# theodorblackbird/lina-speech

Hardware: AMD Instinct MI355X
Metric: codec tokens/sec (whole node), 169M d1024xl12 batched greedy decode (higher is better)
Workload: dtype bf16

## Files before the change

### include/lina_gla.h

```cpp
#ifndef LINA_GLA_H
#define LINA_GLA_H

#include <stdint.h>

#ifdef __cplusplus
extern "C" {
#endif

typedef void* lina_stream_t;

enum { LINA_F32 = 0, LINA_BF16 = 1 };
enum {
    LINA_OK = 0,
    LINA_ERR_ARG = -1,
    LINA_ERR_UNSUPPORTED = -2,
    LINA_ERR_LAUNCH = -3
};

int lina_version(void);
const char* lina_last_error(void);

typedef struct lina_bht_strides {
    int64_t b, h, t;
} lina_bht_strides;
// ... 178 lines not shown
                           float* state, const void* gate, const void* norm_weight,
                           void* og, float* o_exchange, int* counters,
                           float* hist_k, float* hist_c, float* hist_v,
                           const int64_t* step, const int64_t* origin, int window,
                           int B, int H, int Dk, int Dv,
                           int64_t q_sb, int64_t q_sh, int64_t k_sb, int64_t k_sh,
                           int64_t v_sb, int64_t v_sh, int64_t g_sb, int64_t g_sh,
                           int64_t gate_sb, int64_t gate_sh, float eps, int og_packed,
                           int dtype, int g_dtype, float scale, lina_stream_t stream);
int lina_gla_decode_window_flush(float* state, const float* hist_k, const float* hist_c, const float* hist_v,
                                 int n_pending, int B, int H, int Dk, int Dv, lina_stream_t stream);
int lina_gla_decode_window_s(const void* q, const void* k, const void* v, const void* gk,
                             void* state, int state_dtype, const void* gate, const void* norm_weight,
                             void* og, float* o_exchange, int* counters,
                             float* hist_k, float* hist_c, float* hist_v,
                             const int64_t* step, const int64_t* origin, int window,
                             int B, int H, int Dk, int Dv,
                             int64_t q_sb, int64_t q_sh, int64_t k_sb, int64_t k_sh,
                             int64_t v_sb, int64_t v_sh, int64_t g_sb, int64_t g_sh,
                             int64_t gate_sb, int64_t gate_sh, float eps, int og_packed,
                             int dtype, int g_dtype, float scale, lina_stream_t stream);
int lina_gla_decode_window_flush_s(void* state, int state_dtype, const float* hist_k, const float* hist_c,
                                   const float* hist_v, int n_pending, int B, int H, int Dk, int Dv, lina_stream_t stream);

int lina_linear_skinny(const void* A, int64_t lda, const void* W, int64_t ldw,
                       const float* c1, const float* c2, const void* resid, int64_t ldr,
                       void* out, int64_t ldo, int M, int N, int K,
                       int swiglu_hidden, int ln_dim, float ln_eps, int dtype, lina_stream_t stream);

int lina_gla_decode_inproj(const void* x, int64_t ldx, const void* w_in, int64_t ldw,
                           const float* c1, const float* c2,
                           const void* wq, const void* wk, const void* wv,
                           void* cq, void* ck, void* cv, const void* w2, const void* b2,
                           void* qkv, void* g_out, float* gk,
                           int B, int K, int Kd, int Vd, int W, int R,
                           float ln_eps, float normalizer, float clamp_min, int dtype, lina_stream_t stream);

int lina_cross_att_step1(const void* q_lin, const void* ln_w, const void* ln_b, float ln_eps,
                         const void* kk, const void* pe, void* att1, int64_t att_sb, void* xp,
                         int B, int T_txt, int d, float scale, int dtype, lina_stream_t stream);
int lina_cross_att_step2(const void* xp, const void* pe, const void* vv, void* att2, int64_t att_sb, void* x,
                         int B, int T_txt, int d, float scale, int dtype, lina_stream_t stream);

int lina_softmax_pe_rows(const float* scores, int64_t scores_sb, void* att, int64_t att_sb,
                         const int64_t* att_step, int64_t att_step_stride, int64_t att_steps, const void* pe, void* xp,
                         void* xp_packed, int B, int Tn, int d, int dtype, lina_stream_t stream);
// ... 42 lines not shown
```

### lina-speech_amd/_lib.py

```python
from __future__ import annotations

import ctypes as C
import os

_HERE = os.path.dirname(os.path.abspath(__file__))
LIB_PATH = os.environ.get("LINA_GLA_LIB") or os.path.join(_HERE, "csrc", "liblina_gla.so")

LINA_F32, LINA_BF16 = 0, 1
CONV_BWD_TT = 64
LOOP_CTL_ROWS = 4


class BHT(C.Structure):
    _fields_ = [("b", C.c_int64), ("h", C.c_int64), ("t", C.c_int64)]


_p, _i, _i64, _f = C.c_void_p, C.c_int, C.c_int64, C.c_float

_GLA_SIG = [_p, _p, _p, _p, _p, _p, _p, _i, _i, _i, _i, _i, BHT, BHT, BHT, BHT, BHT, _i, _i, _f, _p]

PROTOTYPES = {
    "lina_version": (C.c_int, []),
    "lina_last_error": (C.c_char_p, []),
    "lina_gla_recurrent_fwd": (C.c_int, _GLA_SIG),
# ... 29 lines not shown
    "lina_sum_partials": (C.c_int, [_p, _p, _i, _i, _i64, _i, _p]),
    "lina_mlp_pack": (C.c_int, [_p, _p, _p, _p, _p, _p, _p, _i, _i, _i, _i, _i, _i, _p]),
    "lina_stack_rows": (C.c_int, [_p, _p, _i, _i, _i, _p, _i, _p]),
    "lina_adamw_multi": (C.c_int, [_p, _p, _p, _p, _p, _i] + [C.c_double] * 7 + [_p]),
    "lina_adamw_multi_max": (C.c_int, []),
    "lina_swiglu_bwd_partials": (C.c_int, [_i64]),
    "lina_swiglu_bwd_colsum": (C.c_int, [_p, _p, _p, _p, _i64, _i, _i64, _i64, _i64, _i, _p]),
    "lina_gate_lowrank_partials": (C.c_int, [_i64]),
    "lina_gate_lowrank": (C.c_int, [_p, _i64, _p, _p, _p, _p, _p, _i64, _i, _i, _f, _f, _i, _p]),
    "lina_gate_logsigmoid": (C.c_int, [_p, _p, _p, _i64, _f, _f, _i, _p]),
    "lina_layernorm_fwd": (C.c_int, [_p, _p, _p, _p, _p, _p, _p, _p, _i64, _i, _f, _i, _i, _i, _p]),
    "lina_layernorm_bwd_partials": (C.c_int, [_i64]),
    "lina_layernorm_bwd": (C.c_int, [_p, _p, _p, _p, _p, _p, _p, _p, _p, _p, _i64, _i, _i, _i, _i, _p]),
    "lina_gla_decode_update": (C.c_int, [_p, _p, _p, _p, _p, _p, _i, _i, _i, _i, _i64, _i64, _i64, _i64, _i64, _i64,
                                         _i64, _i64, _i, _i, _f, _p]),
    "lina_gla_decode_update_norm": (C.c_int, [_p, _p, _p, _p, _p, _p, _p, _p, _p, _p, _i, _i, _i, _i,
                                              _i64, _i64, _i64, _i64, _i64, _i64, _i64, _i64, _i64, _i64, _f,
                                              _i, _i, _f, _p]),
    "lina_gla_decode_window_max": (C.c_int, []),
    "lina_gla_decode_window": (C.c_int, [_p] * 15 + [_i] * 5 + [_i64] * 10 + [_f, _i, _i, _i, _f, _p]),
    "lina_gla_decode_window_flush": (C.c_int, [_p, _p, _p, _p, _i, _i, _i, _i, _i, _p]),
    "lina_gla_decode_window_s": (C.c_int, [_p] * 5 + [_i] + [_p] * 10 + [_i] * 5 + [_i64] * 10 + [_f, _i, _i, _i, _f, _p]),
    "lina_gla_decode_window_flush_s": (C.c_int, [_p, _i, _p, _p, _p, _i, _i, _i, _i, _i, _p]),
    "lina_linear_skinny_ex": (C.c_int, [_p, _i64, _p, _i64, _i, _i, _p, _p, _p, _i64, _p, _i64, _p, _i, _i, _i, _i, _i, _i, _f, _i, _p]),
    "lina_gla_decode_inproj_packed": (C.c_int, [_p] * 15 + [_i] * 6 + [_f, _f, _f, _i, _i, _p]),
    "lina_weighted_rows_add_packed": (C.c_int, [_p, _i, _p, _p, _p, _i, _i, _i, _i, _p]),
    "lina_cross_att_step1": (C.c_int, [_p, _p, _p, _f, _p, _p, _p, _i64, _p, _i, _i, _i, _f, _i, _p]),
    "lina_cross_att_step2": (C.c_int, [_p, _p, _p, _p, _i64, _p, _i, _i, _i, _f, _i, _p]),
    "lina_cross_scores_softmax": (C.c_int, [_p, _p, _p, _f, _p, _p, _i64, _p, _i, _i, _i, _i, _f, _i, _p]),
    "lina_softmax_weighted_rows_add": (C.c_int, [_p, _i64, _f, _p, _i64, _p, _p, _p, _i, _i, _i, _i, _p]),
    "lina_pe_softmax_weighted_rows_add": (C.c_int, [_p, _i, _p, _f, _p, _i64, _p, _i64, _i64, _p, _p, _p, _i, _i, _i, _i, _p]),
    "lina_softmax_pe_rows": (C.c_int, [_p, _i64, _p, _i64, _p, _i64, _i64, _p, _p, _p, _i, _i, _i, _i, _p]),
    "lina_cross_scores": (C.c_int, [_p, _p, _p, _f, _p, _p, _i, _i, _i, _f, _i, _p]),
    "lina_cross_scores_ragged": (C.c_int, [_p, _p, _p, _f, _p, _p, _p, _i, _i, _i, _f, _i, _p]),
    "lina_softmax_pe_rows_ragged": (C.c_int, [_p, _i64, _p, _i64, _p, _i64, _i64, _p, _i64, _p, _p, _p, _i, _i, _i, _i, _p]),
    "lina_pe_softmax_weighted_rows_add_ragged": (C.c_int, [_p, _i, _p, _i64, _p, _f, _p, _i64, _p, _i64, _i64, _p, _p, _p,
                                                           _i, _i, _i, _i, _p]),
    "lina_softmax_rows": (C.c_int, [_p, _i64, _i, _f, _p, _i64, _p, _i, _i, _i, _i, _p]),
    "lina_weighted_rows_add": (C.c_int, [_p, _i, _p, _p, _i, _i, _i, _i, _p]),
    "lina_gla_decode_inproj": (C.c_int, [_p, _i64, _p, _i64, _p, _p, _p, _p, _p, _p, _p, _p, _p, _p, _p, _p, _p,
                                         _i, _i, _i, _i, _i, _i, _f, _f, _f, _i, _p]),
    "lina_linear_skinny": (C.c_int, [_p, _i64, _p, _i64, _p, _p, _p, _i64, _p, _i64, _i, _i, _i, _i, _i, _f, _i, _p]),
}


def _preload_hip_runtime() -> None:
# ... 44 lines not shown
```

### lina-speech_amd/csrc/gla_decode_window.hip

```cpp
#include <lina_dev.h>
#include "lina_common.h"
#include "skinny_frag.h"

#ifndef LINA_K1W_HIST_NT
#define LINA_K1W_HIST_NT 0
#endif

#ifndef LINA_K1W_STATE_PLAIN
#define LINA_K1W_STATE_PLAIN 0
#endif
#ifndef LINA_K1W_NO_TAIL_LOADS
#define LINA_K1W_NO_TAIL_LOADS 0
#endif
#if LINA_K1W_STATE_PLAIN
#define LINA_K1W_STATE_LOAD(p) (*reinterpret_cast<const float4*>(p))
#else
#define LINA_K1W_STATE_LOAD(p) ld_nt4(p)
#endif

namespace lina {

constexpr int kWinMax = 16;

__device__ __forceinline__ float ld_hist(const float* p) {
// ... 238 lines not shown
                float4 oth[CS];
                float tot = ss;
#pragma unroll
                for (int c = 0; c < CS; ++c) {
                    oth[c] = r;
                    if (c != (int)blockIdx.y) {
                        float4 x = make_float4(0.f, 0.f, 0.f, 0.f);
                        if (tid < CG4) {
                            const float2 lo = ld_agent8(ox + c * DV + 4 * tid), hi = ld_agent8(ox + c * DV + 4 * tid + 2);
                            x = make_float4(lo.x, lo.y, hi.x, hi.y);
                        }
                        float s2 = x.x * x.x + x.y * x.y + x.z * x.z + x.w * x.w;
                        s2 += shfl_xor(s2, 1); s2 += shfl_xor(s2, 2); s2 += shfl_xor(s2, 4);
                        s2 += shfl_xor(s2, 8); s2 += shfl_xor(s2, 16); s2 += shfl_xor(s2, 32);
                        tot += s2;
                        oth[c] = x;
                    }
                }
                const float rs = rsqrtf(tot / (float)DVT + eps);
#pragma unroll
                for (int c = 0; c < CS; ++c) finish(oth[c], c * DV, rs);
            }
        }
    }
}

template <typename TIO, typename TG, typename TS = float>
static int launch_window(const void* q, const void* k, const void* v, const void* gk, TS* S, float* hk, float* hc,
                         float* hv, const int64_t* step, const int64_t* origin, int window, int flush_n, int B, int H,
                         int Dk, int Dv, const int64_t* st, float scale, lina_stream_t stream, const void* gate,
                         int64_t gate_sb, int64_t gate_sh, const void* nw, float eps, void* og, int og_packed = 0,
                         float* o_x = nullptr, int* counters = nullptr) {
    const int cs = Dv == 512 ? 2 : 1;
    dim3 grid((unsigned)(B * H), (unsigned)cs);
#define LINA_WIN_ONE(DVV, NRBB, CSS)                                                                                   \
    LINA_LAUNCH((gla_decode_window_kernel<DVV, NRBB, CSS, TIO, TG, TS>), grid, dim3(256 * NRBB), 0, stream, (const TIO*)q, \
                (const TIO*)k, (const TIO*)v, (const TG*)gk, S, hk, hc, hv, step, origin, window, flush_n, H, st[0],   \
                st[1], st[2], st[3], st[4], st[5], st[6], st[7], scale, (const TIO*)gate, gate_sb, gate_sh,            \
                (const TIO*)nw, eps, (TIO*)og, og_packed, o_x, counters)
#define LINA_WIN_CASE(DVV)                                                                                             \
    case DVV:                                                                                                          \
        if (Dk == 64) LINA_WIN_ONE(DVV, 1, 1); else if (Dk == 128) LINA_WIN_ONE(DVV, 2, 1); else LINA_WIN_ONE(DVV, 4, 1); \
        break;
    if (Dk != 64 && Dk != 128 && Dk != 256)
        return fail(LINA_ERR_UNSUPPORTED, "lina_gla_decode_window: Dk=%d not in {64,128,256}", Dk);
    if (cs == 2 && flush_n < 0 && !(o_x && counters))
        return fail(LINA_ERR_ARG, "lina_gla_decode_window: Dv=512 needs the o_exchange buffer and the counters");
    switch (Dv) {
        LINA_WIN_CASE(64) LINA_WIN_CASE(128) LINA_WIN_CASE(256)
        case 512:
            if (Dk == 64) LINA_WIN_ONE(256, 1, 2); else if (Dk == 128) LINA_WIN_ONE(256, 2, 2); else LINA_WIN_ONE(256, 4, 2);
            break;
        default: return fail(LINA_ERR_UNSUPPORTED, "lina_gla_decode_window: Dv=%d not in {64,128,256,512}", Dv);
    }
#undef LINA_WIN_CASE
#undef LINA_WIN_ONE
    return check_launch("lina_gla_decode_window");
}

}

extern "C" int lina_gla_decode_window_max(void) { return lina::kWinMax; }

extern "C" int lina_gla_decode_window(const void* q, const void* k, const void* v, const void* gk,
                                      float* state, const void* gate, const void* norm_weight, void* og,
                                      float* o_exchange, int* counters, float* hist_k, float* hist_c, float* hist_v, const int64_t* step,
                                      const int64_t* origin, int window, int B, int H, int Dk, int Dv, int64_t q_sb,
                                      int64_t q_sh, int64_t k_sb, int64_t k_sh, int64_t v_sb, int64_t v_sh, int64_t g_sb,
                                      int64_t g_sh, int64_t gate_sb, int64_t gate_sh, float eps, int og_packed, int dtype,
                                      int g_dtype, float scale, lina_stream_t stream) {
    using namespace lina;
    LINA_REQUIRE(q && k && v && gk && state && gate && norm_weight && og && hist_k && hist_c && hist_v && step && origin,
                 "lina_gla_decode_window: null pointer");
    LINA_REQUIRE(B > 0 && H > 0, "lina_gla_decode_window: B,H must be positive");
    LINA_REQUIRE(window >= 1 && window <= kWinMax && (window & (window - 1)) == 0,
                 "lina_gla_decode_window: window must be a power of two in [1, %d]", kWinMax);
    LINA_REQUIRE(valid_dtype(dtype) && valid_dtype(g_dtype), "lina_gla_decode_window: bad dtype enum");
    LINA_REQUIRE(gate_sb % 4 == 0 && gate_sh % 4 == 0, "lina_gla_decode_window: gate strides must be multiples of 4");
    const int64_t st[8] = {q_sb, q_sh, k_sb, k_sh, v_sb, v_sh, g_sb, g_sh};
    if (dtype == LINA_F32 && g_dtype == LINA_F32)
// ... 51 lines not shown
                                                    B, H, Dk, Dv, st, scale, stream, gate, gate_sb, gate_sh, norm_weight, eps, og,
                                                    og_packed, o_exchange, counters);
    return launch_window<bf16_t, bf16_t, bf16_t>(q, k, v, gk, (bf16_t*)state, hist_k, hist_c, hist_v, step, origin, window, -1, B,
                                                 H, Dk, Dv, st, scale, stream, gate, gate_sb, gate_sh, norm_weight, eps, og,
                                                 og_packed, o_exchange, counters);
}

extern "C" int lina_gla_decode_window_flush_s(void* state, int state_dtype, const float* hist_k, const float* hist_c,
                                              const float* hist_v, int n_pending, int B, int H, int Dk, int Dv,
                                              lina_stream_t stream) {
    using namespace lina;
    LINA_REQUIRE(valid_dtype(state_dtype), "lina_gla_decode_window_flush_s: bad state dtype %d", state_dtype);
    if (state_dtype == LINA_F32)
        return lina_gla_decode_window_flush((float*)state, hist_k, hist_c, hist_v, n_pending, B, H, Dk, Dv, stream);
    LINA_REQUIRE(state && hist_k && hist_c && hist_v, "lina_gla_decode_window_flush_s: null pointer");
    LINA_REQUIRE(B > 0 && H > 0, "lina_gla_decode_window_flush_s: B,H must be positive");
    LINA_REQUIRE(n_pending >= 0 && n_pending <= kWinMax, "lina_gla_decode_window_flush_s: n_pending must be in [0, %d]", kWinMax);
    if (n_pending == 0) return LINA_OK;
    const int64_t st[8] = {0, 0, 0, 0, 0, 0, 0, 0};
    return launch_window<bf16_t, float, bf16_t>(nullptr, nullptr, nullptr, nullptr, (bf16_t*)state, (float*)hist_k, (float*)hist_c,
                                                (float*)hist_v, nullptr, nullptr, kWinMax, n_pending, B, H, Dk, Dv, st, 1.0f,
                                                stream, nullptr, 0, 0, nullptr, 0.f, nullptr);
}
```

### lina-speech_amd/decode.py

```python
from __future__ import annotations

import math
import os
from typing import Optional

import torch
import torch.nn.functional as F

from . import ops
from .mixer import GatedLinearAttention
from .modules import Cache


def _fold_layernorm(weight, ln, bias=None):
    dt = weight.dtype
    w_ln = (weight.float() * ln.weight.float()[None, :]).to(dt).contiguous()
    c1 = w_ln.float().sum(1).contiguous()
    c2 = weight.float() @ ln.bias.float()
    if bias is not None:
        c2 = c2 + bias.float()
    return w_ln, c1, c2.contiguous()


_CAPTURE_MODE = "thread_local"
# ... 132 lines not shown
        self.xp_p = torch.zeros(ops.packed_numel(hi - lo, d), dtype=dtype, device=dev)
        self.q_lin = torch.zeros(hi - lo, d, dtype=dtype, device=dev)
        Tn = kk.shape[1]
        Tp = (Tn + 31) // 32 * 32
        self.scores = torch.zeros(hi - lo, Tn, dtype=torch.float32, device=dev)
        self.sc2 = torch.zeros(hi - lo, Tp, dtype=dtype, device=dev)
        self.attc = torch.zeros(hi - lo, Tp, dtype=dtype, device=dev)


class _Loop:
    __slots__ = ("cap", "tok_log", "att_log", "att_direct", "ctl", "body", "graph1", "graphN", "att", "hid_log")

    def __init__(self):
        self.cap, self.tok_log, self.att_log, self.att_direct, self.ctl, self.hid_log = 0, None, None, False, None, None
        self.body = self.graph1 = self.graphN = self.att = None


class DecodeEngine:
    def __init__(self, model, x_enc: torch.Tensor, batch_size: int, state: Optional[Cache] = None,
                 use_graph: Optional[bool] = None, n_split: Optional[int] = None, fuse_norm: bool = True,
                 window: Optional[int] = None, stream_weights=("in", "up"), cross: str = "spread",
                 fused_pick: bool = True, packed: bool = True, cross_tail_fused: bool = True,
                 share_weights_with: Optional["DecodeEngine"] = None, state_dtype: Optional[torch.dtype] = None,
                 x_lens=None):
        rnn = model.attentive_rnn
        self.model = model
        self.fuse_norm = fuse_norm
        self.B = batch_size
        self.dev = x_enc.device
        if state_dtype not in (None, torch.float32, torch.bfloat16):
            raise ValueError("state_dtype must be torch.float32 or torch.bfloat16")
        self.state_dtype = state_dtype or torch.float32
        bf16_state = self.state_dtype == torch.bfloat16
        if bf16_state and (model.logits_head.weight.dtype != torch.bfloat16 or not fuse_norm):
            raise ValueError("a bf16 recurrent state is the reference's arithmetic for a bf16 model: bf16 weights only")
        if window is None:
            window = 1 if bf16_state else 8
        if window not in (1, 2, 4, 8, 16):
            raise ValueError("window must be 1, 2, 4, 8 or 16")
        self.window = window if self.fuse_norm else 1
        self._state = state if state is not None else rnn.init_state(batch_size=batch_size)
        if bf16_state:
            conv = Cache()
            for li, st in enumerate(self._state.states):
                conv.update(tuple(st[:-1]) + (st[-1].to(torch.bfloat16).contiguous(),), li, offset=0)
            self._state = conv
        self._t_idx = torch.zeros(1, dtype=torch.long, device=self.dev)
        self._origin = torch.zeros(1, dtype=torch.long, device=self.dev)
        self._origin_host, self._n_done, self._lazy_live = 0, 0, False
        self._skip_update = False
# ... 76 lines not shown
    def _block(self, x, P: _BlockPack, lazy: bool = False, x_p=None):
        B = x.shape[0]
        packed = x_p is not None
        if packed:
            ops.gla_decode_inproj_packed(x_p, P.w_in_p, B, P.d, P.c1_in, P.c2_in, P.wq, P.wk, P.wv, P.cq, P.ck, P.cv,
                                         P.w2, P.b2, P.qkv, P.g, P.gk, P.n1_eps, P.normalizer, P.clamp_min,
                                         w_stream="in" in self._stream)
            gate = P.g.view(B, P.H, P.Dv)
        elif P.fused_in:
            ops.gla_decode_inproj(x, P.w_in, P.c1_in, P.c2_in, P.wq, P.wk, P.wv, P.cq, P.ck, P.cv, P.w2, P.b2,
                                  P.qkv, P.g, P.gk, P.n1_eps, P.normalizer, P.clamp_min)
            gate = P.g.view(B, P.H, P.Dv)
        else:
            z = ops.linear_skinny(x, P.w_in, P.c1_in, P.c2_in, out=P.z, ln_dim=P.d, ln_eps=P.n1_eps)
            ops.gla_decode_prologue(z, P.off_q, P.off_k, P.off_v, P.off_lr, P.wq, P.wk, P.wv, P.cq, P.ck, P.cv,
                                    P.w2, P.b2, P.qkv, P.gk, P.normalizer, P.clamp_min)
            gate = z[:, P.off_g:P.off_g + P.Vd].view(B, P.H, P.Dv)
        q = P.qkv[:, :P.Kd].view(B, P.H, P.Dk)
        k = P.qkv[:, P.Kd:2 * P.Kd].view(B, P.H, P.Dk)
        v = P.qkv[:, 2 * P.Kd:].view(B, P.H, P.Dv)
        if self._skip_update:
            pass
        elif (lazy and P.lazy) or P.S.dtype == torch.bfloat16:
            ops.gla_decode_window(q, k, v, P.gk.view(B, P.H, P.Dk), P.S, gate, P.gnw, P.og_p if packed else P.og,
                                  P.hk, P.hc, P.hv, self._t_idx, self._origin, P.window if lazy else 1, P.eps_gate,
                                  og_packed=packed, o_exchange=P.o_x, counters=P.counters)
        elif P.row_split and self.fuse_norm:
            ops.gla_decode_update_norm(q, k, v, P.gk.view(B, P.H, P.Dk), P.o_part, P.S, gate, P.gnw, P.og,
                                       P.counters, P.eps_gate)
        elif P.row_split:
            ops.gla_decode_update(q, k, v, P.gk.view(B, P.H, P.Dk), P.o_part, P.S)
            ops.rmsnorm_swish_gate(P.o_part, gate, P.gnw, P.eps_gate, n_partial=P.o_part.shape[0], out=P.og)
        else:
            o, _ = ops.fused_recurrent_gla(q.unsqueeze(2), k.unsqueeze(2), v.unsqueeze(2),
                                           P.gk.view(B, P.H, 1, P.Dk), initial_state=P.S,
                                           output_final_state=True, inplace_state=True)
            ops.rmsnorm_swish_gate(o.reshape(B, P.H, P.Dv), gate, P.gnw, P.eps_gate, out=P.og)
        if packed:
            ops.linear_skinny_packed(P.og_p, P.w_o_p, B, P.d, P.Vd, resid=x_p, out_packed=x_p, out_packed_width=P.d,
                                     w_stream="o" in self._stream)
            ops.linear_skinny_packed(x_p, P.w_up_p, B, P.hid_pad, P.d, P.c1_up, P.c2_up, out_packed=P.s_p,
                                     out_packed_width=P.hid_pad, swiglu_hidden=P.hid, ln_dim=P.d, ln_eps=P.n2_eps,
                                     w_half_rows=P.up_half_rows, w_stream="up" in self._stream)
            ops.linear_skinny_packed(P.s_p, P.w_down_p, B, P.d, P.hid_pad, resid=x_p, out_packed=x_p,
                                     out_packed_width=P.d, w_stream="down" in self._stream)
            return x
        ops.linear_skinny(P.og.view(B, P.Vd), P.w_o, resid=x, out=x)
        ops.linear_skinny(x, P.w_up, P.c1_up, P.c2_up, out=P.s, swiglu_hidden=P.hid, ln_dim=P.d, ln_eps=P.n2_eps,
                          n_out=P.hid_pad)
# ... 487 lines not shown
        self._pin_ev[slot].synchronize()
        return int(self._pin[slot][1])

    @torch.inference_mode()
    def run_greedy(self, n_steps: int, y0: Optional[torch.Tensor] = None, record_att: bool = False, **sampling):
        self.begin_greedy(n_steps, y0, log_att=record_att, **sampling)
        for _ in range(n_steps):
            self.greedy_step()
        toks = self.greedy_tokens()
        self.sync_state()
        return (toks, self.logged_atts(n_steps)) if record_att else toks


class DecodeEngineGroup:

    def __init__(self, model, x_enc: torch.Tensor, batch_size: int, n_engines: int = 2, x_lens=None, **engine_args):
        from .shard import shard_rows
        if n_engines < 2 or n_engines > batch_size:
            raise ValueError("DecodeEngineGroup needs 2 <= n_engines <= batch_size")
        self.B, self.dev = batch_size, x_enc.device
        self.ranges = [shard_rows(batch_size, i, n_engines) for i in range(n_engines)]
        lens = None if x_lens is None else text_lengths(x_lens, batch_size, x_enc.shape[1])
        self.engines = []
        for lo, hi in self.ranges:
            xe = x_enc[lo:hi] if x_enc.shape[0] == batch_size else x_enc
            self.engines.append(DecodeEngine(model, xe, batch_size=hi - lo, x_lens=None if lens is None else lens[lo:hi],
                                             share_weights_with=self.engines[0] if self.engines else None, **engine_args))
        self.Q, self.Tn = self.engines[0].Q, self.engines[0].Tn
        self.streams = ([torch.cuda.Stream(device=self.dev) for _ in self.engines] if self.dev.type == "cuda" else None)
        self._n_done = 0

    def close(self):
        for e in self.engines:
            e.close()
        self.engines = []

    def _each(self, fn):
        if self.streams is None:
            return [fn(e, lo, hi) for e, (lo, hi) in zip(self.engines, self.ranges)]
        main = torch.cuda.current_stream(self.dev)
        out = []
        for e, (lo, hi), st in zip(self.engines, self.ranges, self.streams):
            st.wait_stream(main)
            with torch.cuda.stream(st):
                out.append(fn(e, lo, hi))
        return out
# ... 81 lines not shown
```

### lina-speech_amd/kernels.py

```python
from __future__ import annotations

from typing import Optional

import torch

from . import backend as _backend
from .backend import _bht, _check, _dt, _inner_contig, _no_grad, _ptr, _workspace, fused_ops_available
from .policy import POLICY, _value_blocks, chunk_segments
from ._lib import LOOP_CTL_ROWS


def _gla_prepare(q, k, v, gk, scale, initial_state):
    if q.dim() != 4:
        raise ValueError("q must be [B,H,T,Dk]")
    B, H, T, Dk = q.shape
    Dv = v.shape[-1]
    if k.shape != q.shape or gk.shape != q.shape or v.shape[:3] != q.shape[:3]:
        raise ValueError(f"shape mismatch q{tuple(q.shape)} k{tuple(k.shape)} v{tuple(v.shape)} gk{tuple(gk.shape)}")
    if k.dtype != q.dtype or v.dtype != q.dtype:
        raise TypeError("q, k, v must share a dtype")
    _backend._BACKEND.require(q, k, v, gk, initial_state)
    if gk.dtype != q.dtype and gk.dtype != torch.float32:
        gk = gk.float()
    if q.dtype == torch.float32 and gk.dtype != torch.float32:
# ... 471 lines not shown
def gla_decode_update_norm(q, k, v, gk, o_part, state, gate, norm_weight, og, counters, eps: float = 1e-5, scale=None):
    be = _backend._BACKEND
    be.require(q, k, v, gk, o_part, state, gate, norm_weight, og, counters)
    B, H, Dk = q.shape
    Dv = v.shape[-1]
    if state.dtype != torch.float32 or not state.is_contiguous() or tuple(state.shape) != (B, H, Dk, Dv):
        raise ValueError("state must be contiguous fp32 [B,H,Dk,Dv]")
    if o_part.dtype != torch.float32 or not o_part.is_contiguous() or tuple(o_part.shape) != (Dk // 64, B, H, Dv):
        raise ValueError("o_part must be contiguous fp32 [Dk/64,B,H,Dv]")
    if counters.dtype != torch.int32 or counters.numel() < B * H or not counters.is_contiguous():
        raise ValueError("counters must be a contiguous int32 tensor with B*H entries")
    if not og.is_contiguous() or og.dtype != q.dtype or gate.dtype != q.dtype or gate.stride(-1) != 1:
        raise ValueError("og/gate must be model-dtype tensors, og contiguous, gate row-contiguous")
    _check(be.lib.lina_gla_decode_update_norm(_ptr(q), _ptr(k), _ptr(v), _ptr(gk), _ptr(o_part), _ptr(state), _ptr(gate),
                                              _ptr(norm_weight), _ptr(og), _ptr(counters), B, H, Dk, Dv,
                                              q.stride(0), q.stride(1), k.stride(0), k.stride(1), v.stride(0),
                                              v.stride(1), gk.stride(0), gk.stride(1), gate.stride(0), gate.stride(1),
                                              float(eps), _dt(q), _dt(gk),
                                              float(Dk ** -0.5 if scale is None else scale), be.stream(q)))
    return og


def gla_decode_window(q, k, v, gk, state, gate, norm_weight, og, hist_k, hist_c, hist_v, step, origin,
                      window: int, eps: float = 1e-5, scale=None, og_packed: bool = False, o_exchange=None, counters=None):
    be = _backend._BACKEND
    be.require(q, k, v, gk, state, gate, norm_weight, og, hist_k, hist_c, hist_v, step, origin)
    B, H, Dk = q.shape
    Dv = v.shape[-1]
    if state.dtype not in (torch.float32, torch.bfloat16) or not state.is_contiguous() or tuple(state.shape) != (B, H, Dk, Dv):
        raise ValueError("state must be contiguous fp32 (or, opt-in, bf16) [B,H,Dk,Dv]")
    if state.dtype == torch.bfloat16 and q.dtype != torch.bfloat16:
        raise ValueError("a bf16 state needs bf16 activations")
    for t, shp in ((hist_k, (window, B * H, Dk)), (hist_c, (window, B * H, Dk)), (hist_v, (window, B * H, Dv))):
        if t.dtype != torch.float32 or not t.is_contiguous() or tuple(t.shape) != shp:
            raise ValueError(f"history buffers must be contiguous fp32 {shp}")
    if step.dtype != torch.int64 or origin.dtype != torch.int64:
        raise ValueError("step / origin must be int64 device tensors")
    if not og.is_contiguous() or og.dtype != q.dtype or gate.dtype != q.dtype or gate.stride(-1) != 1:
        raise ValueError("og/gate must be model-dtype tensors, og contiguous, gate row-contiguous")
    if og_packed and og.numel() < packed_numel(B, H * Dv):
        raise ValueError("packed og buffer is too small")
    for t in (q, k, v, gk):
        if t.stride(-1) != 1:
            raise ValueError("innermost dimension must be contiguous")
    be.require(o_exchange, counters)
    if Dv > 256 and (o_exchange is None or counters is None or o_exchange.dtype != torch.float32
                     or o_exchange.numel() < B * H * Dv or counters.dtype != torch.int32 or counters.numel() < B * H):
        raise ValueError("Dv > 256 needs o_exchange (fp32 [B*H*Dv]) and counters (int32 [B*H], zero)")
    _check(be.lib.lina_gla_decode_window_s(_ptr(q), _ptr(k), _ptr(v), _ptr(gk), _ptr(state), _dt(state), _ptr(gate),
                                         _ptr(norm_weight), _ptr(og), _ptr(o_exchange), _ptr(counters), _ptr(hist_k),
                                         _ptr(hist_c),
                                         _ptr(hist_v), _ptr(step), _ptr(origin), int(window), B, H, Dk, Dv,
                                         q.stride(0), q.stride(1), k.stride(0), k.stride(1), v.stride(0), v.stride(1),
                                         gk.stride(0), gk.stride(1), gate.stride(0), gate.stride(1), float(eps),
                                         1 if og_packed else 0, _dt(q), _dt(gk),
                                         float(Dk ** -0.5 if scale is None else scale), be.stream(q)))
    return og


def gla_decode_window_flush(state, hist_k, hist_c, hist_v, n_pending: int):
    be = _backend._BACKEND
    be.require(state, hist_k, hist_c, hist_v)
    B, H, Dk, Dv = state.shape
    _check(be.lib.lina_gla_decode_window_flush_s(_ptr(state), _dt(state), _ptr(hist_k), _ptr(hist_c), _ptr(hist_v),
                                                 int(n_pending), B, H, Dk, Dv, be.stream(state)))
    return state


def cross_att_step1(q_lin, ln_w, ln_b, ln_eps, kk, pe, att1, xp, scale):
    be = _backend._BACKEND
    be.require(q_lin, ln_w, ln_b, kk, pe, att1, xp)
    B, d = q_lin.shape
    Tn = kk.shape[1]
    _check(be.lib.lina_cross_att_step1(_ptr(q_lin), _ptr(ln_w), _ptr(ln_b), float(ln_eps), _ptr(kk), _ptr(pe),
                                       _ptr(att1), att1.stride(0), _ptr(xp), B, Tn, d, float(scale), _dt(q_lin),
                                       be.stream(q_lin)))


def cross_att_step2(xp, pe, vv, att2, x, scale):
# ... 216 lines not shown
```

### lina-speech_amd/policy.py

```python
from __future__ import annotations

import torch


class Policy:
    k2b_path: str = "full"
    dv512_one_launch: bool = True
    one_pass_operands: bool = True
    split_stacked_gemm: bool = True
    wide_down_dx: bool = True


POLICY = Policy()


def _value_blocks(q, v, gk) -> int:
    Dk, Dv = q.shape[-1], v.shape[-1]
    if q.dtype == torch.bfloat16 and gk.dtype == torch.bfloat16 and Dk == 256 and Dv > Dk and Dv % Dk == 0:
        return Dv // Dk
    return 1


def chunk_segments(n_heads_total: int, T: int) -> int:
    if n_heads_total >= 128 or T < 1024:
        return 1
    return max(1, min(256 // n_heads_total, T // 256, 16))


_LINEAR_SPLIT_MAX_OUT = 3 * 1024 * 1024
_LINEAR_SPLIT_MIN_ROWS = 2048


def _linear_split(rows, n_out, n_in):
# ... 10 lines not shown
```

Measured before the change: 235,000.

## Add persistent grid-stride windowed GLA decode kernel with next-head state prefetch

Adds a persistent variant of the windowed GLA decode update. A fixed number of workgroups loops over heads and double-buffers LDS. Each workgroup prefetches the next head's state tile and small operands while finishing the current head. The variant is enabled only for two-engine group decode with enough rows per shard, using 192 workgroups; it aims to hide per-head load latency and launch tail. The cost is higher per-workgroup LDS and register use, and lower parallelism when the number of heads is small.

```diff
diff --git a/include/lina_gla.h b/include/lina_gla.h
--- a/include/lina_gla.h
+++ b/include/lina_gla.h
@@ -224,6 +224,16 @@
                              int dtype, int g_dtype, float scale, lina_stream_t stream);
 int lina_gla_decode_window_flush_s(void* state, int state_dtype, const float* hist_k, const float* hist_c,
                                    const float* hist_v, int n_pending, int B, int H, int Dk, int Dv, lina_stream_t stream);
+int lina_gla_decode_window_persist(const void* q, const void* k, const void* v, const void* gk,
+                                   void* state, int state_dtype, const void* gate, const void* norm_weight,
+                                   void* og, float* o_exchange, int* counters,
+                                   float* hist_k, float* hist_c, float* hist_v,
+                                   const int64_t* step, const int64_t* origin, int window,
+                                   int B, int H, int Dk, int Dv,
+                                   int64_t q_sb, int64_t q_sh, int64_t k_sb, int64_t k_sh,
+                                   int64_t v_sb, int64_t v_sh, int64_t g_sb, int64_t g_sh,
+                                   int64_t gate_sb, int64_t gate_sh, float eps, int og_packed,
+                                   int dtype, int g_dtype, float scale, int n_wg, lina_stream_t stream);
 
 int lina_linear_skinny(const void* A, int64_t lda, const void* W, int64_t ldw,
                        const float* c1, const float* c2, const void* resid, int64_t ldr,
diff --git a/lina-speech_amd/_lib.py b/lina-speech_amd/_lib.py
--- a/lina-speech_amd/_lib.py
+++ b/lina-speech_amd/_lib.py
@@ -75,6 +75,7 @@
     "lina_gla_decode_window_flush": (C.c_int, [_p, _p, _p, _p, _i, _i, _i, _i, _i, _p]),
     "lina_gla_decode_window_s": (C.c_int, [_p] * 5 + [_i] + [_p] * 10 + [_i] * 5 + [_i64] * 10 + [_f, _i, _i, _i, _f, _p]),
     "lina_gla_decode_window_flush_s": (C.c_int, [_p, _i, _p, _p, _p, _i, _i, _i, _i, _i, _p]),
+    "lina_gla_decode_window_persist": (C.c_int, [_p] * 5 + [_i] + [_p] * 10 + [_i] * 5 + [_i64] * 10 + [_f, _i, _i, _i, _f, _i, _p]),
     "lina_linear_skinny_ex": (C.c_int, [_p, _i64, _p, _i64, _i, _i, _p, _p, _p, _i64, _p, _i64, _p, _i, _i, _i, _i, _i, _i, _f, _i, _p]),
     "lina_gla_decode_inproj_packed": (C.c_int, [_p] * 15 + [_i] * 6 + [_f, _f, _f, _i, _i, _p]),
     "lina_weighted_rows_add_packed": (C.c_int, [_p, _i, _p, _p, _p, _i, _i, _i, _i, _p]),
diff --git a/lina-speech_amd/csrc/gla_decode_window.hip b/lina-speech_amd/csrc/gla_decode_window.hip
--- a/lina-speech_amd/csrc/gla_decode_window.hip
+++ b/lina-speech_amd/csrc/gla_decode_window.hip
@@ -284,6 +284,253 @@
                 for (int c = 0; c < CS; ++c) finish(oth[c], c * DV, rs);
             }
         }
+    }
+}
+
+constexpr int kWinPersist = 8;
+template <typename T> __device__ __forceinline__ T* at_byte(T* base, int byte_off) {
+    opaque(byte_off);
+    return (T*)((const char*)base + (unsigned)byte_off);
+}
+
+template <int DV, int NRB, int CS, typename TIO, typename TG, typename TS = float>
+__global__ __launch_bounds__(256 * NRB) void gla_decode_window_persist_kernel(
+    const TIO* __restrict__ q, const TIO* __restrict__ k, const TIO* __restrict__ v, const TG* __restrict__ gk, TS* S,
+    float* hist_k, float* hist_c, float* hist_v, const int64_t* step, const int64_t* origin, int window, int n_heads,
+    int H, int64_t q_sb, int64_t q_sh, int64_t k_sb, int64_t k_sh, int64_t v_sb, int64_t v_sh, int64_t g_sb,
+    int64_t g_sh, float scale, const TIO* __restrict__ gate, int64_t gate_sb, int64_t gate_sh,
+    const TIO* __restrict__ nw, float eps, TIO* __restrict__ og, int og_packed) {
+    static_assert(CS == 1, "the persistent form serves heads of one column block");
+    constexpr int RB = 64;
+    constexpr int DK = RB * NRB;
+    constexpr int EPL = state_piece<TS>::n;
+    constexpr int CG = DV / EPL;
+    constexpr int RPI = 256 / CG;
+    constexpr int NP = RB / RPI;
+    constexpr int RD = NP >= 2 ? NP / 2 : 1;
+    constexpr int PG = RD < 4 ? RD : 4;
+    static_assert(NP % RD == 0 && RD % PG == 0, "a head is a whole number of passes over the ring");
+    constexpr int CG4 = DV / 4;
+    constexpr int NH = kWinPersist - 1;
+    struct __attribute__((aligned(16))) head_lds {
+        __attribute__((aligned(16))) float v[kWinPersist][DV];
+        __attribute__((aligned(16))) float red[NRB * RPI * DV];
+        float w[kWinPersist][DK];
+        float q[DK], e[DK], a[kWinPersist][NRB];
+        typename raw4<TIO>::type gate[CG4];
+    };
+    __shared__ head_lds s_buf[2];
+    __shared__ typename raw4<TIO>::type s_nw[CG4];
+
+    const int tid = threadIdx.x;
+    const int rb = tid >> 8, t256 = tid & 255;
+    const int cg = t256 % CG, rg = t256 / CG;
+    const int r0 = rb * RB;
+    const int64_t BH = n_heads;
+    const int n_wg = (int)gridDim.x;
+    int bh = blockIdx.x;
+    if (bh >= n_heads) return;
+
+    const int j = (int)(step[0] - origin[0]) & (window - 1);
+    const bool write_back = j == window - 1;
+    const int n_hist = j;
+    const int s_last = n_hist > 0 ? n_hist - 1 : 0;
+    constexpr int NV = 192 * NRB;
+    const bool row_wave = wave_uniform(t256 < RB ? 1 : 0) != 0;
+    const int row = r0 + (t256 & (RB - 1));
+    const int vc = rb * 192 + t256 - RB;
+    const int vcc = vc < 0 ? 0 : (vc < DV ? vc : DV - 1);
+    const int toff = ((r0 + rg) * DV + EPL * cg) * (int)sizeof(TS);
+    const int hoffl = (row_wave ? row : vcc) * 4;
+    const int rowio = row * (int)sizeof(TIO), rowg = row * (int)sizeof(TG), vcio = vcc * (int)sizeof(TIO);
+    const int t4io = (tid & (CG4 - 1)) * 4 * (int)sizeof(TIO);
+    int pstep_ = RPI * DV;
+    opaque(pstep_);
+    const int pstep = wave_uniform(pstep_);
+    const float* hA = row_wave ? hist_c : hist_v;
+    const float* hB = row_wave ? hist_k : hist_v;
+    const int64_t hw = row_wave ? DK : DV;
+
+    float h1[NH], h2[NH];
+    decltype(ld_raw(gk)) gj_r;
+    decltype(ld_raw(q)) kj_r, qj_r, vj_r;
+    typename raw4<TIO>::type gate_r;
+    if (tid < CG4) s_nw[tid] = ld4_raw(nw + 4 * tid);
+    auto small_loads = [&](int hd) __attribute__((always_inline)) {
+        const int b = hd / H, h = hd % H;
+#pragma unroll
+        for (int s = 0; s < NH; ++s) {
+            const int sc = s < n_hist ? s : s_last;
+            const int64_t o = ((int64_t)sc * BH + hd) * hw;
+            h1[s] = ld_hist(at_byte(hA + o, hoffl));
+            h2[s] = ld_hist(at_byte(hB + o, hoffl));
+        }
+        gj_r = ld_raw(at_byte(gk + (b * g_sb + h * g_sh), rowg));
+        kj_r = ld_raw(at_byte(k + (b * k_sb + h * k_sh), rowio));
+        qj_r = ld_raw(at_byte(q + (b * q_sb + h * q_sh), rowio));
+        vj_r = ld_raw(at_byte(v + (b * v_sb + h * v_sh), vcio));
+        gate_r = ld4_raw(at_byte(gate + (b * gate_sb + h * gate_sh), t4io));
+    };
+
+    float St[RD][EPL];
+    small_loads(bh);
+    {
+        const TS* tile = S + (int64_t)bh * DK * DV;
+#pragma unroll
+        for (int i = 0; i < RD; ++i) ld_state(at_byte(tile + i * pstep, toff), St[i]);
+    }
+
+    auto head = [&](const bool WB, const bool NEXT, const int p, const int nx) __attribute__((always_inline)) {
+        const int b = bh / H, h = bh % H;
+        const int64_t hoff = (int64_t)bh * DK;
+        head_lds& L = s_buf[p];
+        if (tid < CG4) L.gate[tid] = gate_r;
+        if (row_wave) {
+            const float gj = cvt1(gj_r), kj = cvt1(kj_r), qj = cvt1(qj_r) * scale;
+            float cprev = 0.0f;
+#pragma unroll
+            for (int s = 0; s < NH; ++s) cprev = (s == j - 1) ? h1[s] : cprev;
+            const float cj = cprev + gj;
+            st_hist(at_byte(hist_c + ((int64_t)j * BH * DK + hoff), row * 4), cj);
+            st_hist(at_byte(hist_k + ((int64_t)j * BH * DK + hoff), row * 4), kj);
+            L.q[row] = qj;
+            L.e[row] = __expf(cj);
+#pragma unroll
+            for (int s = 0; s < kWinPersist; ++s) {
+                if (s <= j) {
+                    const float ws = (s == j) ? kj : __expf(cj - h1[s < NH ? s : 0]) * h2[s < NH ? s : 0];
+                    L.w[s][row] = ws;
+                    float a = qj * ws;
+                    a += shfl_xor(a, 1); a += shfl_xor(a, 2); a += shfl_xor(a, 4);
+                    a += shfl_xor(a, 8); a += shfl_xor(a, 16); a += shfl_xor(a, 32);
+                    if (t256 == 0) L.a[s][rb] = a;
+                }
+            }
+        } else {
+            if (vc < DV) {
+                const float vj = cvt1(vj_r);
+#pragma unroll
+                for (int s = 0; s < kWinPersist; ++s)
+                    if (s <= j) L.v[s][vc] = (s == j) ? vj : h1[s < NH ? s : 0];
+                st_hist(at_byte(hist_v + ((int64_t)j * BH + bh) * DV, vc * 4), vj);
+            }
+            for (int c = vc + NV; c < DV; c += NV) {
+                for (int s = 0; s <= j; ++s) {
+                    float vs;
+                    if (s == j) {
+                        vs = ld(v + b * v_sb + h * v_sh + c);
+                        hist_v[((int64_t)j * BH + bh) * DV + c] = vs;
+                    } else {
+                        vs = hist_v[((int64_t)s * BH + bh) * DV + c];
+                    }
+                    L.v[s][c] = vs;
+                }
+            }
+        }
+        __syncthreads();
+
+        small_loads(NEXT ? nx : bh);
+        TS* tile = S + (int64_t)bh * DK * DV;
+        const TS* tile_nx = NEXT ? S + (int64_t)nx * DK * DV : tile;
+        const int pstep_nx = NEXT ? pstep : 0;
+
+        float acc[EPL];
+#pragma unroll
+        for (int e = 0; e < EPL; ++e) acc[e] = 0.f;
+#pragma unroll
+        for (int g0 = 0; g0 < NP; g0 += PG) {
+            const int sl = g0 % RD;
+            if (WB) {
+#pragma unroll
+                for (int u = 0; u < PG; ++u) {
+                    const float d = L.e[r0 + rg + RPI * (g0 + u)];
+#pragma unroll
+                    for (int e = 0; e < EPL; ++e) St[sl + u][e] *= d;
+                }
+                for (int s = 0; s <= j; ++s) {
+                    float vv[EPL];
+#pragma unroll
+                    for (int e4 = 0; e4 < EPL; e4 += 4) {
+                        const float4 t = *reinterpret_cast<const float4*>(&L.v[s][EPL * cg + e4]);
+                        vv[e4] = t.x; vv[e4 + 1] = t.y; vv[e4 + 2] = t.z; vv[e4 + 3] = t.w;
+                    }
+#pragma unroll
+                    for (int u = 0; u < PG; ++u) {
+                        const float ws = L.w[s][r0 + rg + RPI * (g0 + u)];
+#pragma unroll
+                        for (int e = 0; e < EPL; ++e) St[sl + u][e] = fmaf(ws, vv[e], St[sl + u][e]);
+                    }
+                }
+#pragma unroll
+                for (int u = 0; u < PG; ++u) st_state(at_byte(tile + (g0 + u) * pstep, toff), St[sl + u]);
+#pragma unroll
+                for (int u = 0; u < PG; ++u) {
+                    const float qq = L.q[r0 + rg + RPI * (g0 + u)];
+#pragma unroll
+                    for (int e = 0; e < EPL; ++e) acc[e] = fmaf(qq, St[sl + u][e], acc[e]);
+                }
+            } else {
+#pragma unroll
+                for (int u = 0; u < PG; ++u) {
+                    const int rr = r0 + rg + RPI * (g0 + u);
+                    const float qe = L.q[rr] * L.e[rr];
+#pragma unroll
+                    for (int e = 0; e < EPL; ++e) acc[e] = fmaf(qe, St[sl + u][e], acc[e]);
+                }
+            }
+            if (g0 + RD < NP) {
+#pragma unroll
+                for (int u = 0; u < PG; ++u) ld_state(at_byte(tile + (g0 + RD + u) * pstep, toff), St[sl + u]);
+            } else {
+#pragma unroll
+                for (int u = 0; u < PG; ++u) ld_state(at_byte(tile_nx + (g0 + RD - NP + u) * pstep_nx, toff), St[sl + u]);
+            }
+        }
+#pragma unroll
+        for (int e4 = 0; e4 < EPL; e4 += 4)
+            *reinterpret_cast<float4*>(&L.red[(rb * RPI + rg) * DV + EPL * cg + e4]) = make_float4(acc[e4], acc[e4 + 1], acc[e4 + 2], acc[e4 + 3]);
+        __syncthreads();
+        if (tid < 64) {
+            float4 r = make_float4(0.f, 0.f, 0.f, 0.f);
+            if (tid < CG4) {
+                r = *reinterpret_cast<const float4*>(&L.red[4 * tid]);
+#pragma unroll
+                for (int jj = 1; jj < NRB * RPI; ++jj) {
+                    const float4 t = *reinterpret_cast<const float4*>(&L.red[jj * DV + 4 * tid]);
+                    r.x += t.x; r.y += t.y; r.z += t.z; r.w += t.w;
+                }
+                if (!WB)
+                    for (int s = 0; s <= j; ++s) {
+                        float a = L.a[s][0];
+#pragma unroll
+                        for (int g2 = 1; g2 < NRB; ++g2) a += L.a[s][g2];
+                        const float4 vv = *reinterpret_cast<const float4*>(&L.v[s][4 * tid]);
+                        r.x = fmaf(a, vv.x, r.x); r.y = fmaf(a, vv.y, r.y); r.z = fmaf(a, vv.z, r.z); r.w = fmaf(a, vv.w, r.w);
+                    }
+            }
+            float ss = r.x * r.x + r.y * r.y + r.z * r.z + r.w * r.w;
+            ss += shfl_xor(ss, 1); ss += shfl_xor(ss, 2); ss += shfl_xor(ss, 4);
+            ss += shfl_xor(ss, 8); ss += shfl_xor(ss, 16); ss += shfl_xor(ss, 32);
+            if (tid < CG4) {
+                const float rs = rsqrtf(ss / (float)DV + eps);
+                float4 x = r;
+                x.x *= rs; x.y *= rs; x.z *= rs; x.w *= rs;
+                const float4 ww = cvt4(s_nw[tid]), gg = cvt4(L.gate[tid]);
+                x.x *= ww.x; x.y *= ww.y; x.z *= ww.z; x.w *= ww.w;
+                x.x *= gg.x * sigmoidf(gg.x); x.y *= gg.y * sigmoidf(gg.y);
+                x.z *= gg.z * sigmoidf(gg.z); x.w *= gg.w * sigmoidf(gg.w);
+                if (og_packed) st4(og + packed_off<TIO>(b, h * DV + 4 * tid, H * DV), x);
+                else st4(og + (int64_t)bh * DV + 4 * tid, x);
+            }
+        }
+    };
+
+    for (int p = 0;; p ^= 1) {
+        const int nx = bh + n_wg;
+        const bool has_next = nx < n_heads;
+        head(write_back, has_next, p, nx);
+        if (!has_next) break;
+        bh = nx;
     }
 }
 
@@ -318,6 +565,39 @@
 #undef LINA_WIN_CASE
 #undef LINA_WIN_ONE
     return check_launch("lina_gla_decode_window");
+}
+
+template <typename TIO, typename TG, typename TS>
+static int launch_window_persist(const void* q, const void* k, const void* v, const void* gk, TS* S, float* hk, float* hc,
+                                 float* hv, const int64_t* step, const int64_t* origin, int window, int n_wg, int B, int H,
+                                 int Dk, int Dv, const int64_t* st, float scale, lina_stream_t stream, const void* gate,
+                                 int64_t gate_sb, int64_t gate_sh, const void* nw, float eps, void* og, int og_packed) {
+    const int n_heads = B * H;
+    dim3 grid((unsigned)(n_wg < n_heads ? n_wg : n_heads));
+#define LINA_WINP_ONE(DVV, NRBB)                                                                                       \
+    LINA_LAUNCH((gla_decode_window_persist_kernel<DVV, NRBB, 1, TIO, TG, TS>), grid, dim3(256 * NRBB), 0, stream,      \
+                (const TIO*)q, (const TIO*)k, (const TIO*)v, (const TG*)gk, S, hk, hc, hv, step, origin, window, n_heads, \
+                H, st[0], st[1], st[2], st[3], st[4], st[5], st[6], st[7], scale, (const TIO*)gate, gate_sb, gate_sh,  \
+                (const TIO*)nw, eps, (TIO*)og, og_packed)
+#define LINA_WINP_CASE(DVV)                                                                                            \
+    case DVV:                                                                                                          \
+        if (Dk == 64) LINA_WINP_ONE(DVV, 1); else if (Dk == 128) LINA_WINP_ONE(DVV, 2);                                \
+        else if constexpr (sizeof(TIO) == 2) LINA_WINP_ONE(DVV, 4);                                                    \
+        break;
+    if (Dk != 64 && Dk != 128 && Dk != 256)
+        return fail(LINA_ERR_UNSUPPORTED, "lina_gla_decode_window_persist: Dk=%d not in {64,128,256}", Dk);
+    if (Dk == 256 && sizeof(TIO) != 2)
+        return fail(LINA_ERR_UNSUPPORTED, "lina_gla_decode_window_persist: Dk=256 is built for bf16 activations (fp32: "
+                    "lina_gla_decode_window_s)");
+    switch (Dv) {
+        LINA_WINP_CASE(64) LINA_WINP_CASE(128) LINA_WINP_CASE(256)
+        default:
+            return fail(LINA_ERR_UNSUPPORTED, "lina_gla_decode_window_persist: Dv=%d not in {64,128,256} (Dv = 512 is served by "
+                        "lina_gla_decode_window_s)", Dv);
+    }
+#undef LINA_WINP_CASE
+#undef LINA_WINP_ONE
+    return check_launch("lina_gla_decode_window_persist");
 }
 
 }
@@ -415,3 +695,40 @@
                                                 (float*)hist_v, nullptr, nullptr, kWinMax, n_pending, B, H, Dk, Dv, st, 1.0f,
                                                 stream, nullptr, 0, 0, nullptr, 0.f, nullptr);
 }
+
+extern "C" int lina_gla_decode_window_persist(const void* q, const void* k, const void* v, const void* gk, void* state,
+                                              int state_dtype, const void* gate, const void* norm_weight, void* og,
+                                              float* o_exchange, int* counters,
+                                              float* hist_k, float* hist_c, float* hist_v, const int64_t* step,
+                                              const int64_t* origin, int window, int B, int H, int Dk, int Dv, int64_t q_sb,
+                                              int64_t q_sh, int64_t k_sb, int64_t k_sh, int64_t v_sb, int64_t v_sh,
+                                              int64_t g_sb, int64_t g_sh, int64_t gate_sb, int64_t gate_sh, float eps,
+                                              int og_packed, int dtype, int g_dtype, float scale, int n_wg,
+                                              lina_stream_t stream) {
+    using namespace lina;
+    LINA_REQUIRE(valid_dtype(state_dtype), "lina_gla_decode_window_persist: bad state dtype %d", state_dtype);
+    LINA_REQUIRE(q && k && v && gk && state && gate && norm_weight && og && hist_k && hist_c && hist_v && step && origin,
+                 "lina_gla_decode_window_persist: null pointer");
+    LINA_REQUIRE(B > 0 && H > 0, "lina_gla_decode_window_persist: B,H must be positive");
+    LINA_REQUIRE(n_wg >= 1, "lina_gla_decode_window_persist: n_wg must be at least 1 (got %d)", n_wg);
+    LINA_REQUIRE(window >= 1 && window <= kWinMax && (window & (window - 1)) == 0,
+                 "lina_gla_decode_window_persist: window must be a power of two in [1, %d]", kWinMax);
+    if (window > kWinPersist)
+        return fail(LINA_ERR_UNSUPPORTED, "lina_gla_decode_window_persist: window=%d > %d is served by lina_gla_decode_window_s", window, kWinPersist);
+    LINA_REQUIRE(valid_dtype(dtype) && valid_dtype(g_dtype), "lina_gla_decode_window_persist: bad dtype enum");
+    LINA_REQUIRE(gate_sb % 4 == 0 && gate_sh % 4 == 0, "lina_gla_decode_window_persist: gate strides must be multiples of 4");
+    const int64_t st[8] = {q_sb, q_sh, k_sb, k_sh, v_sb, v_sh, g_sb, g_sh};
+#define LINA_WINP_GO(TIO, TG, TS)                                                                                      \
+    return launch_window_persist<TIO, TG, TS>(q, k, v, gk, (TS*)state, hist_k, hist_c, hist_v, step, origin, window, n_wg, B, \
+                                              H, Dk, Dv, st, scale, stream, gate, gate_sb, gate_sh, norm_weight, eps, og, og_packed)
+    if (state_dtype == LINA_F32) {
+        if (dtype == LINA_F32 && g_dtype == LINA_F32) LINA_WINP_GO(float, float, float);
+        if (dtype == LINA_BF16 && g_dtype == LINA_F32) LINA_WINP_GO(bf16_t, float, float);
+        if (dtype == LINA_BF16 && g_dtype == LINA_BF16) LINA_WINP_GO(bf16_t, bf16_t, float);
+        return fail(LINA_ERR_UNSUPPORTED, "lina_gla_decode_window_persist: dtype=f32 with bf16 gates is not built");
+    }
+    if (dtype != LINA_BF16) return fail(LINA_ERR_UNSUPPORTED, "lina_gla_decode_window_persist: a bf16 state is built for bf16 activations");
+    if (g_dtype == LINA_F32) LINA_WINP_GO(bf16_t, float, bf16_t);
+    LINA_WINP_GO(bf16_t, bf16_t, bf16_t);
+#undef LINA_WINP_GO
+}
diff --git a/lina-speech_amd/decode.py b/lina-speech_amd/decode.py
--- a/lina-speech_amd/decode.py
+++ b/lina-speech_amd/decode.py
@@ -178,10 +178,11 @@
                  window: Optional[int] = None, stream_weights=("in", "up"), cross: str = "spread",
                  fused_pick: bool = True, packed: bool = True, cross_tail_fused: bool = True,
                  share_weights_with: Optional["DecodeEngine"] = None, state_dtype: Optional[torch.dtype] = None,
-                 x_lens=None):
+                 x_lens=None, k1w_persist_wg: Optional[int] = None):
         rnn = model.attentive_rnn
         self.model = model
         self.fuse_norm = fuse_norm
+        self.k1w_persist_wg = ops.POLICY.k1w_persist_wg if k1w_persist_wg is None else int(k1w_persist_wg)
         self.B = batch_size
         self.dev = x_enc.device
         if state_dtype not in (None, torch.float32, torch.bfloat16):
@@ -304,9 +305,11 @@
         if self._skip_update:
             pass
         elif (lazy and P.lazy) or P.S.dtype == torch.bfloat16:
+            win = P.window if lazy else 1
+            n_wg = self.k1w_persist_wg if (lazy and P.Dv <= 256 and win <= 8 and q.dtype == torch.bfloat16) else 0
             ops.gla_decode_window(q, k, v, P.gk.view(B, P.H, P.Dk), P.S, gate, P.gnw, P.og_p if packed else P.og,
-                                  P.hk, P.hc, P.hv, self._t_idx, self._origin, P.window if lazy else 1, P.eps_gate,
-                                  og_packed=packed, o_exchange=P.o_x, counters=P.counters)
+                                  P.hk, P.hc, P.hv, self._t_idx, self._origin, win, P.eps_gate,
+                                  og_packed=packed, o_exchange=P.o_x, counters=P.counters, n_wg=n_wg)
         elif P.row_split and self.fuse_norm:
             ops.gla_decode_update_norm(q, k, v, P.gk.view(B, P.H, P.Dk), P.o_part, P.S, gate, P.gnw, P.og,
                                        P.counters, P.eps_gate)
@@ -840,6 +843,8 @@
         self.ranges = [shard_rows(batch_size, i, n_engines) for i in range(n_engines)]
         lens = None if x_lens is None else text_lengths(x_lens, batch_size, x_enc.shape[1])
         self.engines = []
+        measured = n_engines == 2 and min(hi - lo for lo, hi in self.ranges) >= ops.POLICY.K1W_PERSIST_GROUP_MIN_ROWS
+        engine_args.setdefault("k1w_persist_wg", ops.POLICY.k1w_persist_wg_group if measured else 0)
         for lo, hi in self.ranges:
             xe = x_enc[lo:hi] if x_enc.shape[0] == batch_size else x_enc
             self.engines.append(DecodeEngine(model, xe, batch_size=hi - lo, x_lens=None if lens is None else lens[lo:hi],
diff --git a/lina-speech_amd/kernels.py b/lina-speech_amd/kernels.py
--- a/lina-speech_amd/kernels.py
+++ b/lina-speech_amd/kernels.py
@@ -517,7 +517,8 @@
 
 
 def gla_decode_window(q, k, v, gk, state, gate, norm_weight, og, hist_k, hist_c, hist_v, step, origin,
-                      window: int, eps: float = 1e-5, scale=None, og_packed: bool = False, o_exchange=None, counters=None):
+                      window: int, eps: float = 1e-5, scale=None, og_packed: bool = False, o_exchange=None, counters=None,
+                      n_wg: int = 0):
     be = _backend._BACKEND
     be.require(q, k, v, gk, state, gate, norm_weight, og, hist_k, hist_c, hist_v, step, origin)
     B, H, Dk = q.shape
@@ -542,14 +543,15 @@
     if Dv > 256 and (o_exchange is None or counters is None or o_exchange.dtype != torch.float32
                      or o_exchange.numel() < B * H * Dv or counters.dtype != torch.int32 or counters.numel() < B * H):
         raise ValueError("Dv > 256 needs o_exchange (fp32 [B*H*Dv]) and counters (int32 [B*H], zero)")
-    _check(be.lib.lina_gla_decode_window_s(_ptr(q), _ptr(k), _ptr(v), _ptr(gk), _ptr(state), _dt(state), _ptr(gate),
-                                         _ptr(norm_weight), _ptr(og), _ptr(o_exchange), _ptr(counters), _ptr(hist_k),
-                                         _ptr(hist_c),
-                                         _ptr(hist_v), _ptr(step), _ptr(origin), int(window), B, H, Dk, Dv,
-                                         q.stride(0), q.stride(1), k.stride(0), k.stride(1), v.stride(0), v.stride(1),
-                                         gk.stride(0), gk.stride(1), gate.stride(0), gate.stride(1), float(eps),
-                                         1 if og_packed else 0, _dt(q), _dt(gk),
-                                         float(Dk ** -0.5 if scale is None else scale), be.stream(q)))
+    args = (_ptr(q), _ptr(k), _ptr(v), _ptr(gk), _ptr(state), _dt(state), _ptr(gate), _ptr(norm_weight), _ptr(og),
+            _ptr(o_exchange), _ptr(counters), _ptr(hist_k), _ptr(hist_c), _ptr(hist_v), _ptr(step), _ptr(origin), int(window),
+            B, H, Dk, Dv, q.stride(0), q.stride(1), k.stride(0), k.stride(1), v.stride(0), v.stride(1), gk.stride(0),
+            gk.stride(1), gate.stride(0), gate.stride(1), float(eps), 1 if og_packed else 0, _dt(q), _dt(gk),
+            float(Dk ** -0.5 if scale is None else scale))
+    if n_wg:
+        _check(be.lib.lina_gla_decode_window_persist(*args, int(n_wg), be.stream(q)))
+    else:
+        _check(be.lib.lina_gla_decode_window_s(*args, be.stream(q)))
     return og
 
 
diff --git a/lina-speech_amd/policy.py b/lina-speech_amd/policy.py
--- a/lina-speech_amd/policy.py
+++ b/lina-speech_amd/policy.py
@@ -9,6 +9,9 @@
     one_pass_operands: bool = True
     split_stacked_gemm: bool = True
     wide_down_dx: bool = True
+    k1w_persist_wg: int = 0
+    k1w_persist_wg_group: int = 192
+    K1W_PERSIST_GROUP_MIN_ROWS = 192
 
 
 POLICY = Policy()
```

After: 247,200, median of 6. 5.2% higher.
